# GlassyWing/yolo_deepsort

Measured on AMD Instinct MI355X. Metric: end-to-end frames/sec (detect+ReID+assoc), 608x608, higher is better.
Workload: dtype f16x3

## Files before the change

include/ydsort.h:

```cpp
#ifndef YDSORT_H
#define YDSORT_H

#include <stddef.h>
#include <stdint.h>

#ifdef __cplusplus
extern "C" {
#endif

typedef struct yds_net yds_net;
typedef struct yds_reid yds_reid;
typedef struct yds_trk yds_trk;
typedef struct yds_pipe yds_pipe;
typedef struct yds_comm yds_comm;

int yds_init(int device_id);
int yds_current_device(void);
int yds_device_pci_bus_id(char *buf, int len);
const char *yds_last_error(void);
int yds_device_count(void);
const char *yds_build_info(void);
void *yds_host_alloc(size_t nbytes);
int yds_host_free(void *host);
void *yds_dev_alloc(size_t nbytes);
// ... 13 lines not shown
int yds_darknet_num_boxes(const yds_net *);
int yds_darknet_num_attrs(const yds_net *);
int yds_darknet_num_layers(const yds_net *);
int yds_darknet_layer_shape(const yds_net *, int layer, int *c, int *h, int *w);
int64_t yds_darknet_conv_flops(const yds_net *);
int yds_darknet_forward_f32(yds_net *, const float *nchw_host, int batch, float *out_host);
int yds_darknet_forward_u8(yds_net *, const uint8_t *rgb_hwc_host, int h, int w, int batch,
                           float *out_host_or_null);
int yds_darknet_forward_u8_dev(yds_net *, const uint8_t *rgb_hwc_dev, int h, int w, int batch);
const uint8_t *yds_darknet_last_frames_dev(yds_net *, int *h, int *w, int *batch);
int yds_darknet_layer_output(yds_net *, int layer, int batch, float *nchw_host);
int yds_darknet_get_input(yds_net *, int batch, float *nchw_host);

int yds_nms(yds_net *, int image, float conf_thres, float iou_thres, int frame_h, int frame_w,
            float *out6_host, int cap, int *n_out);
int yds_nms_pred(const float *pred_host, int n_boxes, int attrs, float conf_thres, float iou_thres,
                 float *out6_host, int cap, int *n_out);

int yds_detect_tiled(yds_net *, const uint8_t *rgb_hwc_host, int h, int w, const int32_t *tiles_xyhw, int n_tiles,
                     float conf_thres, float iou_thres, float *out6_host, int cap, int *n_out);
int yds_nms_merge_pred(const float *pred_host, int n_boxes, int attrs, float conf_thres, float iou_thres,
                       float *out6_host, int cap, int *n_out);
int yds_nms_merge_pred_batched(const float *pred_host, int n_frames, int n_boxes, int attrs, float conf_thres, float iou_thres,
                               float *out6_host, int cap, int *n_out);

yds_reid *yds_reid_create(int max_crops);
void yds_reid_destroy(yds_reid *);
int yds_reid_load_tensor(yds_reid *, const char *name, const float *data_host, const int64_t *shape, int ndim);
int yds_reid_finalize(yds_reid *);
int64_t yds_reid_flops_per_crop(void);
// ... 110 lines not shown
```

yolo_deepsort_amd/_lib.py:

```python

from __future__ import annotations

import ctypes as C
import os

import numpy as np

HERE = os.path.dirname(os.path.abspath(__file__))
_TAG = os.environ.get("YDS_BUILD_TAG", "")
LIB_PATH = os.path.join(HERE, "libydsort" + ("_" + _TAG if _TAG else "") + ".so")


class YdsError(RuntimeError):
    pass


_P = C.c_void_p
_I = C.c_int
_F = C.c_float
_SZ = C.c_size_t
_I64 = C.c_int64

SIGNATURES = {
    "yds_init": (_I, [_I]),
# ... 28 lines not shown
    "yds_darknet_last_frames_dev": (_P, [_P, _P, _P, _P]),
    "yds_darknet_layer_output": (_I, [_P, _I, _I, _P]),
    "yds_darknet_get_input": (_I, [_P, _I, _P]),
    "yds_darknet_set_injection": (_I, [_P, _I, _P, _I, _F]),
    "yds_darknet_load_injection_sets": (_I, [_P, _P, _P, _I, _F]),
    "yds_darknet_select_injection_set": (_I, [_P, _I]),
    "yds_conv_variant_name": (C.c_char_p, [_I]),
    "yds_conv_timing_ex": (_I, [_P, _I, _P, _P, _P, _P, _P]),
    "yds_conv_num_variants": (_I, []),
    "yds_conv_clock": (_I, [_P, _P, _I]),
    "yds_set_conv_math": (_I, [_I]),
    "yds_get_conv_math": (_I, []),
    "yds_conv_bench": (_I, [_I, _I, _I, _I, _I, _I, _I, _I, _I, _I, _P, _P]),
    "yds_conv_run": (_I, [_I, _I, _I, _I, _I, _I, _I, _I, _I, _I, _P, _P, _P, _P, _P]),
    "yds_nms": (_I, [_P, _I, _F, _F, _I, _I, _P, _I, _P]),
    "yds_nms_pred": (_I, [_P, _I, _I, _F, _F, _P, _I, _P]),
    "yds_nms_merge_pred": (_I, [_P, _I, _I, _F, _F, _P, _I, _P]),
    "yds_nms_merge_pred_batched": (_I, [_P, _I, _I, _I, _F, _F, _P, _I, _P]),
    "yds_detect_tiled": (_I, [_P, _P, _I, _I, _P, _I, _F, _F, _P, _I, _P]),
    "yds_reid_create": (_P, [_I]),
    "yds_reid_destroy": (None, [_P]),
    "yds_reid_load_tensor": (_I, [_P, C.c_char_p, _P, _P, _I]),
    "yds_reid_finalize": (_I, [_P]),
    "yds_reid_flops_per_crop": (_I64, []),
    "yds_reid_embed": (_I, [_P, _P, _I, _I, _P, _I, _P]),
    "yds_reid_embed_dev": (_I, [_P, _P, _I, _I, _P, _I, _P]),
    "yds_reid_features_dev": (_P, [_P]),
    "yds_reid_preprocess": (_I, [_P, _P, _I, _I, _P, _I, _P]),
    "yds_reid_forward_f32": (_I, [_P, _P, _I, _P]),
    "yds_tracker_create": (_P, [C.c_double, C.c_double, _I, _I, _I]),
# ... 205 lines not shown
```

yolo_deepsort_amd/csrc/common.h:

```cpp
#pragma once
#include <hip/hip_runtime.h>
#include <stdint.h>
#include <stdio.h>
#include <string>
#include <vector>
#include <stdexcept>

namespace yds {

void set_error(const std::string &msg);
struct Error : std::runtime_error {
    explicit Error(const std::string &m) : std::runtime_error(m) {}
};
[[noreturn]] void fail(const char *fmt, ...);
int bound_device();
void bind_thread();
hipStream_t make_stream(bool latency_role);

#define YDS_HIP(expr)                                                                          \
    do {                                                                                       \
        hipError_t _e = (expr);                                                                \
        if (_e != hipSuccess)                                                                  \
            ::yds::fail("%s failed: %s (%s:%d)", #expr, hipGetErrorString(_e), __FILE__, __LINE__); \
    } while (0)
// ... 79 lines not shown
int conv_math();
void set_conv_math(int m);
void pack_weights_f16x3(const float *w, int cout, int kpad, std::vector<uint16_t> &out);
const char *conv_variant_name(int v);
double conv_flops(const ConvArgs &a);
double conv_bytes_io(const View &v);
double conv_bytes(const ConvArgs &a);

void launch_maxpool(const View &x, const View &y, int k, int stride, int pad, bool zero_pad_br, hipStream_t s);
void launch_upsample(const View &x, const View &y, int stride, hipStream_t s);
void launch_copy(const View &x, const View &y, hipStream_t s);
void launch_add(const View &a, const View &b, const View &y, hipStream_t s);
void launch_nchw_to_nhwc(const float *src_nchw, const View &y, int c_src, hipStream_t s);
void launch_nhwc_to_nchw(const View &x, float *dst_nchw, hipStream_t s);
void launch_pack_h16(const float *src_f32, const View &y, hipStream_t s);
void launch_yolo_decode(const View &head, float *out, int total_boxes, int box_off, int num_classes,
                        const float *anchors_wh , int A, int img_h, int img_w, hipStream_t s);
void launch_inject(const View &head, int image, const float *rows_dev, int n, int head_index, int num_classes,
                   float logit, hipStream_t s);
void launch_inject_batch(const View &head, int batch, const float *table_dev, const int *offsets_dev, int max_rows, int head_index,
                         int num_classes, float logit, hipStream_t s);
void launch_resize_u8(const uint8_t *frames, int n, int h, int w, const View &y, hipStream_t s, bool bgr = false);
void launch_window_resize(const uint8_t *frames, int h, int w, const int *tiles_dev, int T, int slot0, int n, const View &y, hipStream_t s,
                          bool bgr);
void launch_window_boxes(const float *pred, int n_boxes, int attrs, const int *tiles_dev, const float *scale_dev, int T, int slot0, int n,
                         float *dst, hipStream_t s);
void launch_crop_resize(const uint8_t *frames, int h, int w, const int *boxes5_dev, int D, const View &y,
                        hipStream_t s, bool bgr = false);
void launch_avgpool_l2norm(const View &x, float *out, hipStream_t s);

// ... 2 lines not shown
```

yolo_deepsort_amd/csrc/darknet.cpp:

```cpp
#include "engine.h"
#include "h16.h"
#include "conv_common.h"

#include <math.h>
#include <stdlib.h>
#include <string.h>
#include <map>
#include <sstream>

namespace yds {

std::vector<CfgBlock> parse_cfg(const std::string &text) {
    std::vector<CfgBlock> blocks;
    std::istringstream in(text);
    std::string line;
    auto strip = [](std::string s) {
        size_t a = s.find_first_not_of(" \t\r\n"), b = s.find_last_not_of(" \t\r\n");
        return a == std::string::npos ? std::string() : s.substr(a, b - a + 1);
    };
    while (std::getline(in, line)) {
        if (line.empty() || line[0] == '#') continue;
        line = strip(line);
        if (line.empty()) fail("cfg: whitespace-only line (the reference parser rejects it too)");
        if (line[0] == '[') {
// ... 277 lines not shown
    plan_half_formats();
    stem_checked_reset();
}

void Darknet::allocate_buffers() {
    size_t total_floats = 0;
    for (size_t i = 0; i < layers.size(); ++i) {
        if (!storage[i].owns) continue;
        const Layer &l = layers[i];
        size_t n = (size_t)batch_max * l.h * l.w * storage[i].ld;
        storage[i].buf.alloc(n);
        YDS_HIP(hipMemsetAsync(storage[i].buf.p, 0, n * sizeof(float), stream));
        total_floats += n;
    }
    input.alloc((size_t)batch_max * img_h * img_w * 4);
    out.alloc((size_t)batch_max * total_boxes * attrs);
    stage_f32.alloc((size_t)batch_max * img_h * img_w * 4);
    activation_bytes = total_floats * sizeof(float);
    YDS_HIP(hipStreamSynchronize(stream));
    inject_rows.clear();
    inject_rows.resize(batch_max);
    inject_n.assign(batch_max, 0);
    inject_active = false;
    inject_offsets.clear();
    inject_set = -1;
    stem_checked = block1_checked = -1;
    stage_n = 0;
}

void Darknet::set_batch_max(int b) {
    if (b < 1) fail("set_batch_max: %d", b);
// ... 21 lines not shown
        return v;
    }
    const Storage &st = storage[r];
    if (st.redirected) {
        const Storage &dst = storage[st.into];
        v.fmt = half_mode ? dst.fmt_half : dst.fmt;
        v.p = dst.buf.p + fmt_slots(v.fmt, st.coff + l.coff);
        v.ld = fmt_slots(v.fmt, dst.ld);
    } else {
        v.fmt = half_mode ? st.fmt_half : st.fmt;
        v.p = st.buf.p + fmt_slots(v.fmt, l.coff);
        v.ld = fmt_slots(v.fmt, st.ld);
    }
    v.p += (size_t)lane_img0 * l.h * l.w * v.ld;
    return v;
}

View Darknet::input_view(int batch) const {
    View v;
    v.p = input.p + (size_t)lane_img0 * img_h * img_w * 4; v.n = batch; v.h = img_h; v.w = img_w; v.c = 4; v.ld = 4;
    return v;
}

size_t Darknet::weight_floats() const {
    size_t n = 0;
    for (const Layer &l : layers)
        if (l.type == "convolutional") n += (size_t)(l.bn ? 4 : 1) * l.c + (size_t)l.c * l.cin_file * l.ksize * l.ksize;
    return n;
}

// ... 212 lines not shown
        } else if (l.type == "route") {
            if (l.refs.size() > 1) {
                View dst = view(i, batch);
                for (auto &cp : l.copies) {
                    View d = dst;
                    d.p += fmt_slots(dst.fmt, cp.second);
                    launch_copy(view(cp.first, batch), d, stream);
                }
            }
        } else if (l.type == "shortcut") {
            if (!l.fused) launch_add(view(l.refs[0], batch), view(l.refs[1], batch), view(i, batch), stream);
        } else if (l.type == "yolo") {
            View head = view(l.src, batch);
            int hidx = 0;
            for (int y : yolo_layers) { if (y == i) break; ++hidx; }
            if (hidx == 0 && out_guard) YDS_HIP(hipStreamWaitEvent(stream, out_guard, 0));
            if (inject_active && inject_set >= 0) {
                launch_inject_batch(head, batch, inject_table.p, inject_offsets_dev.p + (size_t)inject_set * batch_max + first, inject_max_rows, hidx,
                                    l.classes, inject_logit, stream);
            } else {
                for (int b = 0; b < batch && inject_active; ++b)
                    launch_inject(head, b, inject_rows[first + b].p, inject_n[first + b], hidx, l.classes, inject_logit, stream);
            }
            launch_yolo_decode(head, out.p + (size_t)first * total_boxes * attrs, total_boxes, l.box_off, l.classes, l.anchors.data(), (int)l.anchors.size() / 2, img_h, img_w, stream);
        }
    }
}

void Darknet::forward_f32_host(const float *nchw, int batch, float *out_host) {
    size_t n = (size_t)batch * in_channels * img_h * img_w;
    YDS_HIP(hipMemcpyAsync(stage_f32.p, nchw, n * sizeof(float), hipMemcpyHostToDevice, stream));
    launch_nchw_to_nhwc(stage_f32.p, input_view(batch), in_channels, stream);
    run_graph(batch);
    if (out_host) YDS_HIP(hipMemcpyAsync(out_host, out.p, (size_t)batch * total_boxes * attrs * sizeof(float), hipMemcpyDeviceToHost, stream));
    YDS_HIP(hipStreamSynchronize(stream));
}

void Darknet::forward_u8_dev(const uint8_t *frames_dev, int h, int w, int batch) {
    if (in_channels != 3) fail("forward_u8: network expects %d channels", in_channels);
// ... 412 lines not shown
```

yolo_deepsort_amd/csrc/engine.h:

```cpp
#pragma once
#include "common.h"

#include <map>
#include <memory>
#include <string>
#include <utility>
#include <vector>

namespace yds {

struct CfgBlock {
    std::string type;
    std::map<std::string, std::string> kv;
};
std::vector<CfgBlock> parse_cfg(const std::string &text);

struct Layer {
    std::string type;
    int c = 0, h = 0, w = 0;
    int root = -1, coff = 0;
    bool is_view = false;
    int src = -1;
    std::vector<int> refs;
    std::vector<std::pair<int, int>> copies;
// ... 16 lines not shown
    DevBuf<float> buf;
    int ld = 0;
    int fmt = 0;
    int fmt_half = 0;
    bool owns = false;
    bool redirected = false;
    int into = -1, coff = 0;
};

struct WindowTable {
    DevBuf<int> rects;
    DevBuf<float> scale;
    int T = 0;
    void build(const int *rects_xyhw, int n, int img_h, int img_w, hipStream_t s);
    std::vector<float> scale_host;
};

class Darknet {
public:
    Darknet(const std::string &cfg_text, int img_h, int img_w, int batch_max);
    ~Darknet();
    void load_weights(const void *blob, size_t nbytes, int cutoff);
    void set_batch_max(int b);
    void forward_f32_host(const float *nchw, int batch, float *out_host);
    void forward_u8_host(const uint8_t *frames, int h, int w, int batch, float *out_host);
    void forward_u8_dev(const uint8_t *frames_dev, int h, int w, int batch);
    void forward_resized(int batch) { run_graph(batch); }
    bool forward_resized_part(int batch, int part);
    int head_layers() const;
    void forward_tiles_host(const uint8_t *frame, int h, int w, const int *tiles_xyhw, int n_tiles);
// ... 8 lines not shown
    int64_t flops_per_image() const;
    size_t weight_floats() const;
    View view(int layer, int batch) const;
    ConvArgs conv_args(int layer, int batch) const;
    ConvArgs merged_conv_args(int layer, int batch) const;
    View input_view(int batch) const;

    int img_h, img_w, batch_max, in_channels = 3;
    int math = 0;
    bool half_mode = false;
    void stem_checked_reset() { stem_checked = block1_checked = -1; }
    void set_half(bool on);
    void plan_half_formats();
    int owner_of(int layer, int &off) const;
    int total_boxes = 0, attrs = 0;
    std::vector<Layer> layers;
    std::vector<Storage> storage;
    std::vector<int> yolo_layers;
    DevBuf<float> input, out, stage_f32;
    DevBuf<uint8_t> stage_u8;
    int stage_h = 0, stage_w = 0, stage_n = 0;
    DevBuf<float> tiled_pred;
    WindowTable tiles;
    hipStream_t stream = nullptr;
    int32_t header[5] = {0, 0, 0, 0, 0};
    bool weights_loaded = false;
    size_t activation_bytes = 0;
    std::vector<DevBuf<float>> inject_rows;
    std::vector<int> inject_n;
    bool inject_active = false;
// ... 24 lines not shown
    bool block1_fused(int batch);
    hipEvent_t out_guard = nullptr;
    int lane_img0 = 0;
    std::vector<hipStream_t> lane_streams;
    std::vector<hipEvent_t> lane_done;
    hipEvent_t lane_fork = nullptr;
};

class NmsWorkspace {
public:
    explicit NmsWorkspace(int max_candidates = 16384, int frames = 1);
    ~NmsWorkspace();
    NmsWorkspace(const NmsWorkspace &) = delete;
    void launch(const float *pred_dev, size_t pred_stride, int n_frames, int n_boxes, int attrs, float conf_thres, float iou_thres,
                float sx, float sy, int cap, hipStream_t s, bool corner = false, bool merge = false);
    int collect(int frame, float *out6_host, int cap);
    void resize(int max_candidates, int n_frames);
    int needed(int n_frames) const;
    static constexpr int kMaxCandidates = 1 << 18;
    int run(const float *pred_dev, int n_boxes, int attrs, float conf_thres, float iou_thres, float sx, float sy,
            float *out6_host, int cap, hipStream_t s);
    int run_merge(const float *pred_dev, int n_boxes, int attrs, float conf_thres, float iou_thres, float *out6_host, int cap, hipStream_t s);
    int max_cand, frames;
    DevBuf<float> cand;
    DevBuf<float> sorted;
    DevBuf<int> counts;
    DevBuf<int> box_count;
    DevBuf<unsigned long long> mask;
    DevBuf<float> kept;
    DevBuf<int> order;
    int *h_counts = nullptr;
    float *h_kept = nullptr;
};

class ReidNet {
public:
    explicit ReidNet(int max_crops);
    ~ReidNet();
    void load_tensor(const std::string &name, const float *data, const int64_t *shape, int ndim);
    void finalize();
    void embed_dev(const uint8_t *frame_dev, int h, int w, const float *tlwh_host, int D, float *out_host);
    void embed_multi_dev(const uint8_t *frames_dev, int h, int w, const float *tlwh_host, const int *frame_of, int D, bool bgr = false);
    void embed_host(const uint8_t *frame_host, int h, int w, const float *tlwh_host, int D, float *out_host);
    void preprocess_host(const uint8_t *frame_host, int h, int w, const float *tlwh_host, int D, float *nchw_host);
    void forward_f32_host(const float *nchw, int D, float *out_host);
    void forward(int D);
    void reserve(int D);
// ... 48 lines not shown
```

yolo_deepsort_amd/csrc/layers.hip:

```cpp
#include "common.h"

#include <algorithm>
#include "h16.h"

namespace yds {

static inline int grid_for(size_t work, int block = 256) {
    size_t g = (work + block - 1) / block;
    if (g > 8192) g = 8192;
    if (g < 1) g = 1;
    return (int)g;
}

__global__ void maxpool_kernel(const float *x, float *y, int N, int H, int W, int C, int ldx, int Ho, int Wo, int ldy,
                               int k, int stride, int pad, int zero_br, int fmt_in, int fmt_out) {
    fp16_saturate_on();
    const int C4 = C >> 2;
    const size_t total = (size_t)N * Ho * Wo * C4;
    for (size_t idx = blockIdx.x * (size_t)blockDim.x + threadIdx.x; idx < total; idx += (size_t)gridDim.x * blockDim.x) {
        int c4 = idx % C4;
        size_t pix = idx / C4;
        int ox = pix % Wo;
        size_t t = pix / Wo;
        int oy = t % Ho;
// ... 147 lines not shown
        const float v[4] = {t.x, t.y, t.z, t.w};
        h16_store4(y + pix * ldy, c4 * 4, v);
    }
}
void launch_pack_h16(const float *src_f32, const View &y, hipStream_t s) {
    if (y.c % 32 || y.ld % 32) fail("pack_h16: channels must be a multiple of 32");
    hipLaunchKernelGGL(pack_h16_kernel, dim3(grid_for(y.pixels() * (y.c / 4))), dim3(256), 0, s, src_f32, y.p, y.pixels(), y.c, y.ld);
    YDS_HIP(hipGetLastError());
}

void launch_nhwc_to_nchw(const View &x, float *dst_nchw, hipStream_t s) {
    hipLaunchKernelGGL(nhwc_to_nchw_kernel, dim3(grid_for(x.pixels() * x.c)), dim3(256), 0, s, x.p, dst_nchw, x.n, x.c, x.h, x.w, x.ld, x.fmt);
    YDS_HIP(hipGetLastError());
}

struct YoloParams {
    float aw[8], ah[8];
    float s0, s1;
};

__global__ void yolo_decode_kernel(const float *head, float *out, int N, int H, int W, int ld, int A, int attrs, int total_boxes,
                                   int box_off, YoloParams yp) {
    const int HW = H * W, n = blockIdx.y, per_cell = A * attrs;
    (void)N;
    const int lane = threadIdx.x & 63;
    const int wave0 = __builtin_amdgcn_readfirstlane((int)((blockIdx.x * blockDim.x + threadIdx.x) >> 6));
    const int nwaves = (int)((gridDim.x * blockDim.x) >> 6);
    for (int cell = wave0; cell < HW; cell += nwaves) {
        const int gy = cell / W, gx = cell - gy * W;
        const float *src = head + ((size_t)(n * H + gy) * W + gx) * ld;
        float *dst = out + ((size_t)n * total_boxes + box_off + cell) * attrs;
        for (int i = lane; i < per_cell; i += 64) {
            int a = 0;
#pragma unroll
            for (int k = 1; k < 8; ++k) a += (k < A && i >= k * attrs) ? 1 : 0;
            const int t = i - a * attrs;
            const float v = src[i];
            float r;
            if (t == 0) r = __fmul_rn(__fadd_rn(1.f / (1.f + expf(-v)), (float)gx), yp.s0);
            else if (t == 1) r = __fmul_rn(__fadd_rn(1.f / (1.f + expf(-v)), (float)gy), yp.s1);
            else if (t == 2) r = __fmul_rn(__fmul_rn(expf(v), yp.aw[a]), yp.s0);
            else if (t == 3) r = __fmul_rn(__fmul_rn(expf(v), yp.ah[a]), yp.s1);
            else r = 1.f / (1.f + expf(-v));
            dst[(size_t)a * HW * attrs + t] = r;
        }
    }
}

void launch_yolo_decode(const View &head, float *out, int total_boxes, int box_off, int num_classes, const float *anchors_wh,
                        int A, int img_h, int img_w, hipStream_t s) {
    if (A > 8) fail("yolo: at most 8 anchors per head");
    YoloParams yp;
    yp.s0 = (float)((double)img_h / head.h);
    yp.s1 = (float)((double)img_w / head.w);
    for (int a = 0; a < A; ++a) {
        yp.aw[a] = anchors_wh[2 * a] / yp.s0;
        yp.ah[a] = anchors_wh[2 * a + 1] / yp.s1;
    }
    int attrs = num_classes + 5;
    if (head.c != A * attrs) fail("yolo: head has %d channels, expected %d", head.c, A * attrs);
    const size_t per_img = (size_t)A * head.h * head.w * attrs;
    if (per_img >= (1ull << 31)) fail("yolo: head too large for 32-bit indexing");
    const unsigned cells = (unsigned)head.h * head.w;
    hipLaunchKernelGGL(yolo_decode_kernel, dim3(std::min((cells + 3) / 4, 2048u), head.n), dim3(256), 0, s, head.p, out, head.n, head.h, head.w,
                       head.ld, A, attrs, total_boxes, box_off, yp);
    YDS_HIP(hipGetLastError());
}

__global__ void inject_clear_kernel(float *head, int image, int H, int W, int ld, int A, int attrs, float logit) {
    int total = H * W * A;
    for (int idx = blockIdx.x * blockDim.x + threadIdx.x; idx < total; idx += gridDim.x * blockDim.x) {
        int a = idx % A, cell = idx / A;
        head[((size_t)image * H * W + cell) * ld + a * attrs + 4] = -logit;
// ... 255 lines not shown
```

yolo_deepsort_amd/csrc/nms.hip:

```cpp
#include "engine.h"

#include <string.h>

#include <algorithm>
#include <vector>

namespace yds {

constexpr int MAX_DET = 300;

__global__ void nms_count_kernel(const float *pred_all, size_t pred_stride, int n_boxes, int attrs, float thr, int *box_count_all) {
    const float *pred = pred_all + blockIdx.y * pred_stride;
    int *box_count = box_count_all + (size_t)blockIdx.y * n_boxes;
    int i = blockIdx.x * blockDim.x + threadIdx.x;
    if (i >= n_boxes) return;
    const float *p = pred + (size_t)i * attrs;
    int cnt = 0;
    float obj = p[4];
    if (obj > thr) {
        for (int j = 5; j < attrs; ++j) cnt += __fmul_rn(p[j], obj) > thr;
    }
    box_count[i] = cnt;
}

__global__ void nms_scan_kernel(int *box_count_all, int n_boxes, int *counts_all) {
    int *box_count = box_count_all + (size_t)blockIdx.y * n_boxes;
    int *counts = counts_all + blockIdx.y * 4;
    __shared__ int wave_sum[16];
    __shared__ int carry;
    const int tid = threadIdx.x, lane = tid & 63, wave = tid >> 6;
    if (tid == 0) carry = 0;
    __syncthreads();
    for (int base = 0; base < n_boxes; base += blockDim.x) {
        int i = base + tid;
        int v = i < n_boxes ? box_count[i] : 0;
// ... 3 lines not shown
            if (lane >= o) incl += t;
        }
        if (lane == 63) wave_sum[wave] = incl;
        __syncthreads();
        int woff = 0;
        for (int w = 0; w < wave; ++w) woff += wave_sum[w];
        int c = carry;
        if (i < n_boxes) box_count[i] = c + woff + incl - v;
        __syncthreads();
        if (tid == (int)blockDim.x - 1) carry = c + woff + incl;
        __syncthreads();
    }
    if (tid == 0) { counts[0] = carry; counts[1] = 0; }
}

__global__ void nms_emit_kernel(const float *pred_all, size_t pred_stride, int n_boxes, int attrs, float thr, const int *box_off_all, int max_cand,
                                float *cand_all, int corner) {
    const float *pred = pred_all + blockIdx.y * pred_stride;
    const int *box_off = box_off_all + (size_t)blockIdx.y * n_boxes;
    float *cand = cand_all + (size_t)blockIdx.y * max_cand * 6;
    int i = blockIdx.x * blockDim.x + threadIdx.x;
    if (i >= n_boxes) return;
    const float *p = pred + (size_t)i * attrs;
    float obj = p[4];
    if (!(obj > thr)) return;
    int slot = box_off[i];
    float x1 = p[0], y1 = p[1], x2 = p[2], y2 = p[3];
    if (!corner) {
        float hw = __fdiv_rn(p[2], 2.f), hh = __fdiv_rn(p[3], 2.f);
        x1 = __fsub_rn(p[0], hw); y1 = __fsub_rn(p[1], hh); x2 = __fadd_rn(p[0], hw); y2 = __fadd_rn(p[1], hh);
    }
    for (int j = 5; j < attrs; ++j) {
        float sc = __fmul_rn(p[j], obj);
        if (sc > thr) {
            if (slot < max_cand) {
                float *r = cand + (size_t)slot * 6;
                r[0] = x1; r[1] = y1; r[2] = x2; r[3] = y2; r[4] = sc; r[5] = (float)(j - 5);
            }
            ++slot;
        }
    }
}

__global__ void nms_rank_kernel(const float *cand_all, const int *counts_all, int max_cand, float *sorted_all) {
    const float *cand = cand_all + (size_t)blockIdx.y * max_cand * 6;
    float *sorted = sorted_all + (size_t)blockIdx.y * max_cand * 6;
    const int *counts = counts_all + blockIdx.y * 4;
    __shared__ float tile[256];
// ... 158 lines not shown
        mean[threadIdx.x] = __fdiv_rn((float)acc, wsum);
    }
    __syncthreads();
    for (int i = threadIdx.x; i < k * 4; i += blockDim.x) kept[(size_t)(i >> 2) * 6 + (i & 3)] = mean[i & 3];
}

__global__ __launch_bounds__(256) void nms_publish_kernel(const int *counts, const float *kept, int *h_counts, float *h_kept, int cap) {
    const int f = blockIdx.x;
    if (threadIdx.x < 4) h_counts[f * 4 + threadIdx.x] = counts[f * 4 + threadIdx.x];
    const int n = min(counts[f * 4 + 1], cap) * 6;
    const float *src = kept + (size_t)f * MAX_DET * 6;
    float *dst = h_kept + (size_t)f * MAX_DET * 6;
    for (int i = threadIdx.x; i < n; i += 256) dst[i] = src[i];
}

void NmsWorkspace::launch(const float *pred_dev, size_t pred_stride, int n_frames, int n_boxes, int attrs, float conf_thres, float iou_thres,
                          float sx, float sy, int cap, hipStream_t s, bool corner, bool merge) {
    if (attrs < 6) fail("nms: predictions need at least one class");
    if (n_frames < 1) fail("nms: no frames");
    if (n_frames > frames) resize(max_cand, n_frames);
    box_count.ensure((size_t)frames * n_boxes);
    const int nb = (n_boxes + 255) / 256;
    hipLaunchKernelGGL(nms_count_kernel, dim3(nb, n_frames), dim3(256), 0, s, pred_dev, pred_stride, n_boxes, attrs, conf_thres, box_count.p);
    hipLaunchKernelGGL(nms_scan_kernel, dim3(1, n_frames), dim3(1024), 0, s, box_count.p, n_boxes, counts.p);
    hipLaunchKernelGGL(nms_emit_kernel, dim3(nb, n_frames), dim3(256), 0, s, pred_dev, pred_stride, n_boxes, attrs, conf_thres, box_count.p,
                       max_cand, cand.p, corner ? 1 : 0);
    hipLaunchKernelGGL(nms_rank_kernel, dim3(16, n_frames), dim3(256), 0, s, cand.p, counts.p, max_cand, sorted.p);
    const int words_ld = max_cand / 64;
    hipLaunchKernelGGL(nms_mask_kernel, dim3(64, n_frames), dim3(256), 0, s, sorted.p, counts.p, max_cand, (double)iou_thres, mask.p, words_ld);
    hipLaunchKernelGGL(nms_sweep_kernel, dim3(1, n_frames), dim3(256), words_ld * sizeof(unsigned long long), s, sorted.p, mask.p, words_ld,
                       counts.p, max_cand, sx, sy, kept.p, cap);
    if (merge) hipLaunchKernelGGL(nms_merge_kernel, dim3(n_frames), dim3(256), 0, s, cand.p, sorted.p, counts.p, max_cand, iou_thres, kept.p);
    hipLaunchKernelGGL(nms_publish_kernel, dim3(n_frames), dim3(256), 0, s, counts.p, kept.p, h_counts, h_kept, std::min(cap, (int)MAX_DET));
    YDS_HIP(hipGetLastError());
}

int NmsWorkspace::collect(int frame, float *out6_host, int cap) {
    const int *c = h_counts + frame * 4;
    if (c[0] > max_cand) fail("nms: %d candidates exceed the workspace capacity %d (caller must resize and relaunch)", c[0], max_cand);
    int n = c[1] < cap ? c[1] : cap;
    if (n > 0) memcpy(out6_host, h_kept + (size_t)frame * MAX_DET * 6, (size_t)n * 6 * sizeof(float));
    return n;
}

int NmsWorkspace::run(const float *pred_dev, int n_boxes, int attrs, float conf_thres, float iou_thres, float sx, float sy,
                      float *out6_host, int cap, hipStream_t s) {
    launch(pred_dev, 0, 1, n_boxes, attrs, conf_thres, iou_thres, sx, sy, cap, s);
    YDS_HIP(hipStreamSynchronize(s));
    if (needed(1) > max_cand) {
// ... 54 lines not shown
yds::NmsWorkspace &workspace() {
    static thread_local std::unique_ptr<yds::NmsWorkspace> ws;
    if (!ws) ws.reset(new yds::NmsWorkspace());
    return *ws;
}
}

extern "C" {

int yds_nms(yds_net *n, int image, float conf_thres, float iou_thres, int frame_h, int frame_w, float *out6_host, int cap, int *n_out) {
    YDS_API_BEGIN
    yds::Darknet *d = n->d;
    if (image < 0 || image >= d->batch_max) yds::fail("nms: image %d outside batch", image);
    float sx = frame_h > 0 ? (float)((double)frame_w / d->img_w) : 1.f;
    float sy = frame_h > 0 ? (float)((double)frame_h / d->img_h) : 1.f;
    const float *pred = d->out.p + (size_t)image * d->total_boxes * d->attrs;
    *n_out = workspace().run(pred, d->total_boxes, d->attrs, conf_thres, iou_thres, sx, sy, out6_host, cap, d->stream);
    YDS_API_END
}

int yds_detect_tiled(yds_net *n, const uint8_t *rgb_hwc_host, int h, int w, const int32_t *tiles_xyhw, int n_tiles, float conf_thres,
                     float iou_thres, float *out6_host, int cap, int *n_out) {
    YDS_API_BEGIN
    yds::Darknet *d = n->d;
    d->forward_tiles_host(rgb_hwc_host, h, w, tiles_xyhw, n_tiles);
    *n_out = workspace().run_merge(d->tiled_pred.p, n_tiles * d->total_boxes, d->attrs, conf_thres, iou_thres, out6_host, cap, d->stream);
    YDS_API_END
}

int yds_nms_merge_pred(const float *pred_host, int n_boxes, int attrs, float conf_thres, float iou_thres, float *out6_host, int cap, int *n_out) {
    YDS_API_BEGIN
    yds::DevBuf<float> pred;
// ... 37 lines not shown
```

yolo_deepsort_amd/csrc/pipeline.cpp:

```cpp
#include "engine.h"

#include <limits.h>
#include <stdlib.h>

#include <chrono>
#include <utility>

namespace yds {

struct DetSlot {
    std::unique_ptr<NmsWorkspace> nms;
    hipEvent_t e0, e1, e2, e_nms;
    hipEvent_t e_r0, e_r1;
    bool reid_in_pass = false;
    DetSlot() { for (hipEvent_t *e : {&e0, &e1, &e2, &e_nms, &e_r0, &e_r1}) YDS_HIP(hipEventCreate(e)); }
    ~DetSlot() { for (hipEvent_t e : {e0, e1, e2, e_nms, e_r0, e_r1}) (void)hipEventDestroy(e); }
};

struct Pass {
    const uint8_t *frames = nullptr;
    int h = 0, w = 0, batch = 0;
    int slot = 0;
    enum { NOTHING, HEAD, WHOLE } done = NOTHING;
    bool split = false;
// ... 73 lines not shown
        hipEvent_t up_done = nullptr;
        Read rd[2];
        Slot() { for (hipEvent_t *e : {&up_done, &rd[DET].ev, &rd[REID].ev}) YDS_HIP(hipEventCreateWithFlags(e, hipEventDisableTiming)); }
        ~Slot() { for (hipEvent_t e : {up_done, rd[DET].ev, rd[REID].ev}) (void)hipEventDestroy(e); }
    };
    Slot slots[N];
    int turn = 0;
    hipStream_t copy_stream = nullptr, det_stream, reid_stream;
};

class Pipeline {
public:
    Pipeline(Darknet *net, ReidNet *reid, std::vector<TrackerIface *> trks, bool multi, float conf, float nms_iou, const int32_t *mask, int n_mask)
        : net(net), reid(reid), trks(std::move(trks)), group(make_tracker_group()), multi(multi), conf(conf), nms_thres(nms_iou),
          class_mask(mask, mask + n_mask), deep_min(getenv("YDS_PIPE_DEEP_MIN") ? atoi(getenv("YDS_PIPE_DEEP_MIN")) : 64),
          stager(net->stream, reid->stream) {
        for (DetSlot &s : det) s.nms.reset(new NmsWorkspace(4096, net->batch_max));
        YDS_HIP(hipEventCreateWithFlags(&ev_feat, hipEventDisableTiming));
        YDS_HIP(hipEventCreateWithFlags(&ev_reid_done, hipEventDisableTiming));
    }
    ~Pipeline() {
        (void)hipEventDestroy(ev_feat);
        (void)hipEventDestroy(ev_reid_done);
    }

    void prefetch_host(const uint8_t *frames_host, int h, int w, int batch) {
        if (stager.find(frames_host) >= 0) return;
        stager.upload(frames_host, (size_t)batch * h * w * 3, 3, stager.cur, stager.next);
    }
    void step_host(const uint8_t *frames_host, const uint8_t *next_host, int h, int w, int batch, int32_t *out6, int cap, int32_t *counts) {
// ... 28 lines not shown
    }
    void launch_detector_tail(Pass &p) {
        DetSlot &s = det[p.slot];
        const size_t per_slot = (size_t)net->total_boxes * net->attrs;
        if (const int T = windows_for(p.h, p.w)) {
            if (win_pred.n < (size_t)p.batch * T * per_slot) {
                YDS_HIP(hipStreamSynchronize(net->stream));
                win_pred.alloc((size_t)p.batch * T * per_slot);
            }
            net->forward_windows(p.frames, p.h, p.w, p.batch, win, win_pred.p, frames_bgr);
            stager.mark_read(p.frames, net->stream, FrameStager::DET);
            YDS_HIP(hipEventRecord(s.e2, net->stream));
            s.nms->launch(win_pred.p, (size_t)T * per_slot, p.batch, T * net->total_boxes, net->attrs, conf, nms_thres, 1.f, 1.f, 300, net->stream,
                          true, true);
        } else {
            if (p.split) (void)net->forward_resized_part(p.batch, 1);
            else net->forward_resized(p.batch);
            YDS_HIP(hipEventRecord(s.e2, net->stream));
            const float sx = (float)((double)p.w / net->img_w), sy = (float)((double)p.h / net->img_h);
            s.nms->launch(net->out.p, per_slot, p.batch, net->total_boxes, net->attrs, conf, nms_thres, sx, sy, 300, net->stream);
        }
        YDS_HIP(hipEventRecord(s.e_nms, net->stream));
        p.done = Pass::WHOLE;
    }

    void set_windows(int ww, int wh, double overlap) {
        if (pending.frames || ahead.reid_in_flight) fail("pipeline: set_windows while a look-ahead pass is in flight (consume it with a step first)");
        if (ww > 0 && wh <= 0) fail("pipeline: window %d x %d", ww, wh);
        if (ww > 0 && !(overlap >= 0)) fail("pipeline: window overlap %g", overlap);
        win_w = ww > 0 ? ww : 0; win_h = ww > 0 ? wh : 0; win_overlap = overlap;
        win_tab_h = win_tab_w = 0;
    }
    int windows_for(int h, int w) {
        if (win_w <= 0 || (w < win_w && h < win_h)) return 0;
        if (h == win_tab_h && w == win_tab_w) return win.T;
// ... 172 lines not shown
        for (int b = 0; b < n; ++b)
            if (stream_of_frame[b] < 0 || stream_of_frame[b] >= (int)trks.size())
                fail("pipeline: frame %d belongs to stream %d outside [0,%zu)", b, stream_of_frame[b], trks.size());
        stream_of.assign(stream_of_frame, stream_of_frame + n);
    }

    Darknet *net;
    ReidNet *reid;
    std::vector<TrackerIface *> trks;
    std::unique_ptr<TrackerGroupIface> group;
    const bool multi;
    std::vector<int32_t> stream_of;
    float conf, nms_thres;
    std::vector<int32_t> class_mask;
    const int deep_min;
    DetSlot det[2];
    Pass pending;
    FrameStager stager;
    Dets cur, ahead;
    DevBuf<float> feat_cur;
    int next_inject_set = -1;
    hipEvent_t ev_feat = nullptr;
    int schedule_min_crops = INT_MIN;
    Trial trials[2];
    hipEvent_t ev_reid_done = nullptr;
    hipStream_t reid_last_on = nullptr;
    bool last_serial = false;
    bool frames_bgr = false;
    float stage_us[5] = {0, 0, 0, 0, 0};
    int win_w = 0, win_h = 0, win_tab_h = 0, win_tab_w = 0;
// ... 111 lines not shown
```

yolo_deepsort_amd/models.py:

```python

from __future__ import annotations

import ctypes as C

import numpy as np

from . import _lib
from .loaders import parse_model_config


def _to_numpy(x):
    if hasattr(x, "detach"):
        x = x.detach().cpu().numpy()
    return np.ascontiguousarray(x, dtype=np.float32)


class _Param:

    def __init__(self, device):
        self.device = device


class Darknet:
    def __init__(self, config_path, img_size=416, batch_max=1, cfg_text=None):
# ... 107 lines not shown
            self.set_batch_max(b)
        out = np.empty((b, self.num_boxes, self.num_attrs), np.float32) if want_output else None
        _lib.check(_lib.load().yds_darknet_forward_u8(self._h, _lib.ptr(frames), h, w, b, _lib.ptr(out)))
        return out

    def last_frame_dev(self, frame):
        if getattr(self, "_last_frame_src", None) is not frame:
            return None
        h, w, b = C.c_int(), C.c_int(), C.c_int()
        p = _lib.load().yds_darknet_last_frames_dev(self._h, C.byref(h), C.byref(w), C.byref(b))
        if not p or b.value != 1 or (h.value, w.value) != tuple(frame.shape[:2]):
            return None
        return C.c_void_p(p)

    def nms(self, image, conf_thres, iou_thres, frame_hw=None, cap=300):
        out = np.empty((cap, 6), np.float32)
        n = C.c_int(0)
        fh, fw = frame_hw if frame_hw is not None else (0, 0)
        _lib.check(_lib.load().yds_nms(self._h, image, conf_thres, iou_thres, fh, fw, _lib.ptr(out), cap, C.byref(n)))
        return out[:n.value].copy()

    def detect_tiled(self, frame, tiles, conf_thres, iou_thres, cap=300):
        frame = np.ascontiguousarray(frame, dtype=np.uint8)
        h, w, _ = frame.shape
        rects = np.ascontiguousarray(tiles, dtype=np.int32).reshape(-1, 4)
        out = np.empty((cap, 6), np.float32)
        n = C.c_int(0)
        _lib.check(_lib.load().yds_detect_tiled(self._h, _lib.ptr(frame), h, w, _lib.ptr(rects), rects.shape[0], conf_thres, iou_thres,
                                                _lib.ptr(out), cap, C.byref(n)))
        return out[:n.value].copy()

    def layer_shape(self, i):
        c, h, w = C.c_int(), C.c_int(), C.c_int()
        _lib.check(_lib.load().yds_darknet_layer_shape(self._h, i, C.byref(c), C.byref(h), C.byref(w)))
# ... 48 lines not shown
```

Measured before the change: 1675.

## Fuse YOLO head decode into NMS candidate kernels, skipping dense decode buffer

```diff
diff --git a/include/ydsort.h b/include/ydsort.h
--- a/include/ydsort.h
+++ b/include/ydsort.h
@@ -51,6 +51,8 @@
 
 int yds_nms(yds_net *, int image, float conf_thres, float iou_thres, int frame_h, int frame_w,
             float *out6_host, int cap, int *n_out);
+int yds_nms_heads(yds_net *, int image, float conf_thres, float iou_thres, int frame_h, int frame_w,
+                  float *out6_host, int cap, int *n_out);
 int yds_nms_pred(const float *pred_host, int n_boxes, int attrs, float conf_thres, float iou_thres,
                  float *out6_host, int cap, int *n_out);
 
diff --git a/yolo_deepsort_amd/_lib.py b/yolo_deepsort_amd/_lib.py
--- a/yolo_deepsort_amd/_lib.py
+++ b/yolo_deepsort_amd/_lib.py
@@ -66,6 +66,7 @@
     "yds_conv_bench": (_I, [_I, _I, _I, _I, _I, _I, _I, _I, _I, _I, _P, _P]),
     "yds_conv_run": (_I, [_I, _I, _I, _I, _I, _I, _I, _I, _I, _I, _P, _P, _P, _P, _P]),
     "yds_nms": (_I, [_P, _I, _F, _F, _I, _I, _P, _I, _P]),
+    "yds_nms_heads": (_I, [_P, _I, _F, _F, _I, _I, _P, _I, _P]),
     "yds_nms_pred": (_I, [_P, _I, _I, _F, _F, _P, _I, _P]),
     "yds_nms_merge_pred": (_I, [_P, _I, _I, _F, _F, _P, _I, _P]),
     "yds_nms_merge_pred_batched": (_I, [_P, _I, _I, _I, _F, _F, _P, _I, _P]),
diff --git a/yolo_deepsort_amd/csrc/common.h b/yolo_deepsort_amd/csrc/common.h
--- a/yolo_deepsort_amd/csrc/common.h
+++ b/yolo_deepsort_amd/csrc/common.h
@@ -117,6 +117,11 @@
 void launch_nchw_to_nhwc(const float *src_nchw, const View &y, int c_src, hipStream_t s);
 void launch_nhwc_to_nchw(const View &x, float *dst_nchw, hipStream_t s);
 void launch_pack_h16(const float *src_f32, const View &y, hipStream_t s);
+struct YoloParams {
+    float aw[8], ah[8];
+    float s0, s1;
+};
+YoloParams yolo_params(const View &head, const float *anchors_wh , int A, int img_h, int img_w);
 void launch_yolo_decode(const View &head, float *out, int total_boxes, int box_off, int num_classes,
                         const float *anchors_wh , int A, int img_h, int img_w, hipStream_t s);
 void launch_inject(const View &head, int image, const float *rows_dev, int n, int head_index, int num_classes,
diff --git a/yolo_deepsort_amd/csrc/darknet.cpp b/yolo_deepsort_amd/csrc/darknet.cpp
--- a/yolo_deepsort_amd/csrc/darknet.cpp
+++ b/yolo_deepsort_amd/csrc/darknet.cpp
@@ -315,7 +315,8 @@
         total_floats += n;
     }
     input.alloc((size_t)batch_max * img_h * img_w * 4);
-    out.alloc((size_t)batch_max * total_boxes * attrs);
+    out.release();
+    heads_written = false;
     stage_f32.alloc((size_t)batch_max * img_h * img_w * 4);
     activation_bytes = total_floats * sizeof(float);
     YDS_HIP(hipStreamSynchronize(stream));
@@ -367,6 +368,23 @@
     }
     v.p += (size_t)lane_img0 * l.h * l.w * v.ld;
     return v;
+}
+
+bool Darknet::head_table(YoloHeads &t) const {
+    t = YoloHeads();
+    if (yolo_layers.empty() || (int)yolo_layers.size() > YoloHeads::kMax) return false;
+    for (int y : yolo_layers) {
+        const Layer &l = layers[y];
+        View v = view(l.src, 1);
+        const int A = (int)l.anchors.size() / 2;
+        if (v.fmt != FMT_F32 || A > 8 || v.c != A * attrs) return false;
+        v.p -= (size_t)lane_img0 * l.h * l.w * v.ld;
+        YoloHead &h = t.head[t.n++];
+        h.p = v.p; h.h = v.h; h.w = v.w; h.ld = v.ld; h.A = A; h.box_off = l.box_off;
+        h.yp = yolo_params(v, l.anchors.data(), A, img_h, img_w);
+    }
+    t.attrs = attrs; t.total_boxes = total_boxes;
+    return true;
 }
 
 View Darknet::input_view(int batch) const {
@@ -609,7 +627,7 @@
             View head = view(l.src, batch);
             int hidx = 0;
             for (int y : yolo_layers) { if (y == i) break; ++hidx; }
-            if (hidx == 0 && out_guard) YDS_HIP(hipStreamWaitEvent(stream, out_guard, 0));
+            if (decode_dense && hidx == 0 && out_guard) YDS_HIP(hipStreamWaitEvent(stream, out_guard, 0));
             if (inject_active && inject_set >= 0) {
                 launch_inject_batch(head, batch, inject_table.p, inject_offsets_dev.p + (size_t)inject_set * batch_max + first, inject_max_rows, hidx,
                                     l.classes, inject_logit, stream);
@@ -617,7 +635,11 @@
                 for (int b = 0; b < batch && inject_active; ++b)
                     launch_inject(head, b, inject_rows[first + b].p, inject_n[first + b], hidx, l.classes, inject_logit, stream);
             }
-            launch_yolo_decode(head, out.p + (size_t)first * total_boxes * attrs, total_boxes, l.box_off, l.classes, l.anchors.data(), (int)l.anchors.size() / 2, img_h, img_w, stream);
+            if (decode_dense) {
+                out.ensure((size_t)batch_max * total_boxes * attrs);
+                launch_yolo_decode(head, out.p + (size_t)first * total_boxes * attrs, total_boxes, l.box_off, l.classes, l.anchors.data(), (int)l.anchors.size() / 2, img_h, img_w, stream);
+            }
+            heads_written = true;
         }
     }
 }
diff --git a/yolo_deepsort_amd/csrc/engine.h b/yolo_deepsort_amd/csrc/engine.h
--- a/yolo_deepsort_amd/csrc/engine.h
+++ b/yolo_deepsort_amd/csrc/engine.h
@@ -54,6 +54,17 @@
     int T = 0;
     void build(const int *rects_xyhw, int n, int img_h, int img_w, hipStream_t s);
     std::vector<float> scale_host;
+};
+
+struct YoloHead {
+    const float *p = nullptr;
+    int h = 0, w = 0, ld = 0, A = 0, box_off = 0;
+    YoloParams yp;
+};
+struct YoloHeads {
+    static constexpr int kMax = 4;
+    YoloHead head[kMax];
+    int n = 0, attrs = 0, total_boxes = 0;
 };
 
 class Darknet {
@@ -92,6 +103,9 @@
     void plan_half_formats();
     int owner_of(int layer, int &off) const;
     int total_boxes = 0, attrs = 0;
+    bool decode_dense = true;
+    bool heads_written = false;
+    bool head_table(YoloHeads &t) const;
     std::vector<Layer> layers;
     std::vector<Storage> storage;
     std::vector<int> yolo_layers;
@@ -146,6 +160,7 @@
     NmsWorkspace(const NmsWorkspace &) = delete;
     void launch(const float *pred_dev, size_t pred_stride, int n_frames, int n_boxes, int attrs, float conf_thres, float iou_thres,
                 float sx, float sy, int cap, hipStream_t s, bool corner = false, bool merge = false);
+    void launch_heads(const YoloHeads &heads, int n_frames, float conf_thres, float iou_thres, float sx, float sy, int cap, hipStream_t s);
     int collect(int frame, float *out6_host, int cap);
     void resize(int max_candidates, int n_frames);
     int needed(int n_frames) const;
@@ -163,6 +178,10 @@
     DevBuf<int> order;
     int *h_counts = nullptr;
     float *h_kept = nullptr;
+
+private:
+    template <class Src> void launch_from(const Src &src, int n_frames, float conf_thres, float iou_thres, float sx, float sy, int cap,
+                                          hipStream_t s, bool corner, bool merge);
 };
 
 class ReidNet {
diff --git a/yolo_deepsort_amd/csrc/layers.hip b/yolo_deepsort_amd/csrc/layers.hip
--- a/yolo_deepsort_amd/csrc/layers.hip
+++ b/yolo_deepsort_amd/csrc/layers.hip
@@ -2,6 +2,7 @@
 
 #include <algorithm>
 #include "h16.h"
+#include "yolo_decode.h"
 
 namespace yds {
 
@@ -185,11 +186,6 @@
     YDS_HIP(hipGetLastError());
 }
 
-struct YoloParams {
-    float aw[8], ah[8];
-    float s0, s1;
-};
-
 __global__ void yolo_decode_kernel(const float *head, float *out, int N, int H, int W, int ld, int A, int attrs, int total_boxes,
                                    int box_off, YoloParams yp) {
     const int HW = H * W, n = blockIdx.y, per_cell = A * attrs;
@@ -207,27 +203,26 @@
             for (int k = 1; k < 8; ++k) a += (k < A && i >= k * attrs) ? 1 : 0;
             const int t = i - a * attrs;
             const float v = src[i];
-            float r;
-            if (t == 0) r = __fmul_rn(__fadd_rn(1.f / (1.f + expf(-v)), (float)gx), yp.s0);
-            else if (t == 1) r = __fmul_rn(__fadd_rn(1.f / (1.f + expf(-v)), (float)gy), yp.s1);
-            else if (t == 2) r = __fmul_rn(__fmul_rn(expf(v), yp.aw[a]), yp.s0);
-            else if (t == 3) r = __fmul_rn(__fmul_rn(expf(v), yp.ah[a]), yp.s1);
-            else r = 1.f / (1.f + expf(-v));
-            dst[(size_t)a * HW * attrs + t] = r;
+            dst[(size_t)a * HW * attrs + t] = yolo_decode_value(t, v, gx, gy, a, yp);
         }
     }
 }
 
-void launch_yolo_decode(const View &head, float *out, int total_boxes, int box_off, int num_classes, const float *anchors_wh,
-                        int A, int img_h, int img_w, hipStream_t s) {
+YoloParams yolo_params(const View &head, const float *anchors_wh, int A, int img_h, int img_w) {
     if (A > 8) fail("yolo: at most 8 anchors per head");
-    YoloParams yp;
+    YoloParams yp = {};
     yp.s0 = (float)((double)img_h / head.h);
     yp.s1 = (float)((double)img_w / head.w);
     for (int a = 0; a < A; ++a) {
         yp.aw[a] = anchors_wh[2 * a] / yp.s0;
         yp.ah[a] = anchors_wh[2 * a + 1] / yp.s1;
     }
+    return yp;
+}
+
+void launch_yolo_decode(const View &head, float *out, int total_boxes, int box_off, int num_classes, const float *anchors_wh,
+                        int A, int img_h, int img_w, hipStream_t s) {
+    const YoloParams yp = yolo_params(head, anchors_wh, A, img_h, img_w);
     int attrs = num_classes + 5;
     if (head.c != A * attrs) fail("yolo: head has %d channels, expected %d", head.c, A * attrs);
     const size_t per_img = (size_t)A * head.h * head.w * attrs;
diff --git a/yolo_deepsort_amd/csrc/nms.hip b/yolo_deepsort_amd/csrc/nms.hip
--- a/yolo_deepsort_amd/csrc/nms.hip
+++ b/yolo_deepsort_amd/csrc/nms.hip
@@ -1,4 +1,5 @@
 #include "engine.h"
+#include "yolo_decode.h"
 
 #include <string.h>
 
@@ -9,16 +10,53 @@
 
 constexpr int MAX_DET = 300;
 
-__global__ void nms_count_kernel(const float *pred_all, size_t pred_stride, int n_boxes, int attrs, float thr, int *box_count_all) {
-    const float *pred = pred_all + blockIdx.y * pred_stride;
+struct DenseRows {
+    const float *pred;
+    size_t stride;
+    int n_boxes, n_attrs;
+    struct Row {
+        const float *p;
+        __device__ __forceinline__ float obj() const { return p[4]; }
+        __device__ __forceinline__ float cls(int j) const { return p[j]; }
+        __device__ __forceinline__ float box(int k) const { return p[k]; }
+    };
+    __host__ __device__ __forceinline__ int boxes() const { return n_boxes; }
+    __host__ __device__ __forceinline__ int attrs() const { return n_attrs; }
+    __device__ __forceinline__ Row row(int frame, int i) const { return Row{pred + frame * stride + (size_t)i * n_attrs}; }
+};
+struct HeadRows {
+    YoloHeads t;
+    struct Row {
+        const float *p;
+        const YoloHead *head;
+        int gx, gy, a;
+        __device__ __forceinline__ float obj() const { return yolo_sigmoid(p[4]); }
+        __device__ __forceinline__ float cls(int j) const { return yolo_sigmoid(p[j]); }
+        __device__ __forceinline__ float box(int k) const { return yolo_decode_value(k, p[k], gx, gy, a, head->yp); }
+    };
+    __host__ __device__ __forceinline__ int boxes() const { return t.total_boxes; }
+    __host__ __device__ __forceinline__ int attrs() const { return t.attrs; }
+    __device__ __forceinline__ Row row(int frame, int i) const {
+        int h = 0;
+#pragma unroll
+        for (int k = 1; k < YoloHeads::kMax; ++k) h += (k < t.n && i >= t.head[k].box_off) ? 1 : 0;
+        const YoloHead *hd = &t.head[h];
+        const int HW = hd->h * hd->w, r = i - hd->box_off;
+        const int a = r / HW, cell = r - a * HW, gy = cell / hd->w;
+        return Row{hd->p + ((size_t)frame * HW + cell) * hd->ld + a * t.attrs, hd, cell - gy * hd->w, gy, a};
+    }
+};
+
+template <class Src> __global__ void nms_count_kernel(Src src, float thr, int *box_count_all) {
+    const int n_boxes = src.boxes(), attrs = src.attrs();
     int *box_count = box_count_all + (size_t)blockIdx.y * n_boxes;
     int i = blockIdx.x * blockDim.x + threadIdx.x;
     if (i >= n_boxes) return;
-    const float *p = pred + (size_t)i * attrs;
+    const typename Src::Row p = src.row(blockIdx.y, i);
     int cnt = 0;
-    float obj = p[4];
+    float obj = p.obj();
     if (obj > thr) {
-        for (int j = 5; j < attrs; ++j) cnt += __fmul_rn(p[j], obj) > thr;
+        for (int j = 5; j < attrs; ++j) cnt += __fmul_rn(p.cls(j), obj) > thr;
     }
     box_count[i] = cnt;
 }
@@ -52,24 +90,24 @@
     if (tid == 0) { counts[0] = carry; counts[1] = 0; }
 }
 
-__global__ void nms_emit_kernel(const float *pred_all, size_t pred_stride, int n_boxes, int attrs, float thr, const int *box_off_all, int max_cand,
-                                float *cand_all, int corner) {
-    const float *pred = pred_all + blockIdx.y * pred_stride;
+template <class Src> __global__ void nms_emit_kernel(Src src, float thr, const int *box_off_all, int max_cand, float *cand_all, int corner) {
+    const int n_boxes = src.boxes(), attrs = src.attrs();
     const int *box_off = box_off_all + (size_t)blockIdx.y * n_boxes;
     float *cand = cand_all + (size_t)blockIdx.y * max_cand * 6;
     int i = blockIdx.x * blockDim.x + threadIdx.x;
     if (i >= n_boxes) return;
-    const float *p = pred + (size_t)i * attrs;
-    float obj = p[4];
+    const typename Src::Row p = src.row(blockIdx.y, i);
+    float obj = p.obj();
     if (!(obj > thr)) return;
     int slot = box_off[i];
-    float x1 = p[0], y1 = p[1], x2 = p[2], y2 = p[3];
+    const float b0 = p.box(0), b1 = p.box(1), b2 = p.box(2), b3 = p.box(3);
+    float x1 = b0, y1 = b1, x2 = b2, y2 = b3;
     if (!corner) {
-        float hw = __fdiv_rn(p[2], 2.f), hh = __fdiv_rn(p[3], 2.f);
-        x1 = __fsub_rn(p[0], hw); y1 = __fsub_rn(p[1], hh); x2 = __fadd_rn(p[0], hw); y2 = __fadd_rn(p[1], hh);
+        float hw = __fdiv_rn(b2, 2.f), hh = __fdiv_rn(b3, 2.f);
+        x1 = __fsub_rn(b0, hw); y1 = __fsub_rn(b1, hh); x2 = __fadd_rn(b0, hw); y2 = __fadd_rn(b1, hh);
     }
     for (int j = 5; j < attrs; ++j) {
-        float sc = __fmul_rn(p[j], obj);
+        float sc = __fmul_rn(p.cls(j), obj);
         if (sc > thr) {
             if (slot < max_cand) {
                 float *r = cand + (size_t)slot * 6;
@@ -258,17 +296,17 @@
     for (int i = threadIdx.x; i < n; i += 256) dst[i] = src[i];
 }
 
-void NmsWorkspace::launch(const float *pred_dev, size_t pred_stride, int n_frames, int n_boxes, int attrs, float conf_thres, float iou_thres,
-                          float sx, float sy, int cap, hipStream_t s, bool corner, bool merge) {
+template <class Src> void NmsWorkspace::launch_from(const Src &src, int n_frames, float conf_thres, float iou_thres, float sx, float sy, int cap,
+                                                    hipStream_t s, bool corner, bool merge) {
+    const int n_boxes = src.boxes(), attrs = src.attrs();
     if (attrs < 6) fail("nms: predictions need at least one class");
     if (n_frames < 1) fail("nms: no frames");
     if (n_frames > frames) resize(max_cand, n_frames);
     box_count.ensure((size_t)frames * n_boxes);
     const int nb = (n_boxes + 255) / 256;
-    hipLaunchKernelGGL(nms_count_kernel, dim3(nb, n_frames), dim3(256), 0, s, pred_dev, pred_stride, n_boxes, attrs, conf_thres, box_count.p);
+    hipLaunchKernelGGL(nms_count_kernel<Src>, dim3(nb, n_frames), dim3(256), 0, s, src, conf_thres, box_count.p);
     hipLaunchKernelGGL(nms_scan_kernel, dim3(1, n_frames), dim3(1024), 0, s, box_count.p, n_boxes, counts.p);
-    hipLaunchKernelGGL(nms_emit_kernel, dim3(nb, n_frames), dim3(256), 0, s, pred_dev, pred_stride, n_boxes, attrs, conf_thres, box_count.p,
-                       max_cand, cand.p, corner ? 1 : 0);
+    hipLaunchKernelGGL(nms_emit_kernel<Src>, dim3(nb, n_frames), dim3(256), 0, s, src, conf_thres, box_count.p, max_cand, cand.p, corner ? 1 : 0);
     hipLaunchKernelGGL(nms_rank_kernel, dim3(16, n_frames), dim3(256), 0, s, cand.p, counts.p, max_cand, sorted.p);
     const int words_ld = max_cand / 64;
     hipLaunchKernelGGL(nms_mask_kernel, dim3(64, n_frames), dim3(256), 0, s, sorted.p, counts.p, max_cand, (double)iou_thres, mask.p, words_ld);
@@ -277,6 +315,16 @@
     if (merge) hipLaunchKernelGGL(nms_merge_kernel, dim3(n_frames), dim3(256), 0, s, cand.p, sorted.p, counts.p, max_cand, iou_thres, kept.p);
     hipLaunchKernelGGL(nms_publish_kernel, dim3(n_frames), dim3(256), 0, s, counts.p, kept.p, h_counts, h_kept, std::min(cap, (int)MAX_DET));
     YDS_HIP(hipGetLastError());
+}
+
+void NmsWorkspace::launch(const float *pred_dev, size_t pred_stride, int n_frames, int n_boxes, int attrs, float conf_thres, float iou_thres,
+                          float sx, float sy, int cap, hipStream_t s, bool corner, bool merge) {
+    launch_from(DenseRows{pred_dev, pred_stride, n_boxes, attrs}, n_frames, conf_thres, iou_thres, sx, sy, cap, s, corner, merge);
+}
+
+void NmsWorkspace::launch_heads(const YoloHeads &heads, int n_frames, float conf_thres, float iou_thres, float sx, float sy, int cap, hipStream_t s) {
+    if (heads.n < 1 || heads.n > YoloHeads::kMax) fail("nms: head table of %d yolo layers", heads.n);
+    launch_from(HeadRows{heads}, n_frames, conf_thres, iou_thres, sx, sy, cap, s, false, false);
 }
 
 int NmsWorkspace::collect(int frame, float *out6_host, int cap) {
@@ -361,8 +409,30 @@
     if (image < 0 || image >= d->batch_max) yds::fail("nms: image %d outside batch", image);
     float sx = frame_h > 0 ? (float)((double)frame_w / d->img_w) : 1.f;
     float sy = frame_h > 0 ? (float)((double)frame_h / d->img_h) : 1.f;
+    if (!d->out.p) yds::fail("nms: this network has not run a dense decode (no forward yet, or only passes that left the head tensors: yds_nms_heads)");
     const float *pred = d->out.p + (size_t)image * d->total_boxes * d->attrs;
     *n_out = workspace().run(pred, d->total_boxes, d->attrs, conf_thres, iou_thres, sx, sy, out6_host, cap, d->stream);
+    YDS_API_END
+}
+
+int yds_nms_heads(yds_net *n, int image, float conf_thres, float iou_thres, int frame_h, int frame_w, float *out6_host, int cap, int *n_out) {
+    YDS_API_BEGIN
+    yds::Darknet *d = n->d;
+    if (image < 0 || image >= d->batch_max) yds::fail("nms: image %d outside batch", image);
+    yds::YoloHeads heads;
+    if (!d->head_table(heads)) yds::fail("nms: this network's heads are read through the dense decode only (yds_nms)");
+    if (!d->heads_written) yds::fail("nms: this network has not run a forward yet (its head tensors hold nothing)");
+    for (int h = 0; h < heads.n; ++h) heads.head[h].p += (size_t)image * heads.head[h].h * heads.head[h].w * heads.head[h].ld;
+    float sx = frame_h > 0 ? (float)((double)frame_w / d->img_w) : 1.f;
+    float sy = frame_h > 0 ? (float)((double)frame_h / d->img_h) : 1.f;
+    yds::NmsWorkspace &ws = workspace();
+    for (int pass = 0; pass < 2; ++pass) {
+        ws.launch_heads(heads, 1, conf_thres, iou_thres, sx, sy, cap, d->stream);
+        YDS_HIP(hipStreamSynchronize(d->stream));
+        if (ws.needed(1) <= ws.max_cand) break;
+        ws.resize(ws.needed(1), ws.frames);
+    }
+    *n_out = ws.collect(0, out6_host, cap);
     YDS_API_END
 }
 
diff --git a/yolo_deepsort_amd/csrc/pipeline.cpp b/yolo_deepsort_amd/csrc/pipeline.cpp
--- a/yolo_deepsort_amd/csrc/pipeline.cpp
+++ b/yolo_deepsort_amd/csrc/pipeline.cpp
@@ -111,6 +111,7 @@
     Pipeline(Darknet *net, ReidNet *reid, std::vector<TrackerIface *> trks, bool multi, float conf, float nms_iou, const int32_t *mask, int n_mask)
         : net(net), reid(reid), trks(std::move(trks)), group(make_tracker_group()), multi(multi), conf(conf), nms_thres(nms_iou),
           class_mask(mask, mask + n_mask), deep_min(getenv("YDS_PIPE_DEEP_MIN") ? atoi(getenv("YDS_PIPE_DEEP_MIN")) : 64),
+          dense_decode(getenv("YDS_DENSE_DECODE") && atoi(getenv("YDS_DENSE_DECODE")) != 0),
           stager(net->stream, reid->stream) {
         for (DetSlot &s : det) s.nms.reset(new NmsWorkspace(4096, net->batch_max));
         YDS_HIP(hipEventCreateWithFlags(&ev_feat, hipEventDisableTiming));
@@ -169,11 +170,18 @@
             s.nms->launch(win_pred.p, (size_t)T * per_slot, p.batch, T * net->total_boxes, net->attrs, conf, nms_thres, 1.f, 1.f, 300, net->stream,
                           true, true);
         } else {
-            if (p.split) (void)net->forward_resized_part(p.batch, 1);
-            else net->forward_resized(p.batch);
+            YoloHeads heads;
+            const bool sparse = !dense_decode && net->head_table(heads);
+            {
+                struct Restore { bool &v; bool keep; ~Restore() { v = keep; } } restore{net->decode_dense, net->decode_dense};
+                net->decode_dense = !sparse;
+                if (p.split) (void)net->forward_resized_part(p.batch, 1);
+                else net->forward_resized(p.batch);
+            }
             YDS_HIP(hipEventRecord(s.e2, net->stream));
             const float sx = (float)((double)p.w / net->img_w), sy = (float)((double)p.h / net->img_h);
-            s.nms->launch(net->out.p, per_slot, p.batch, net->total_boxes, net->attrs, conf, nms_thres, sx, sy, 300, net->stream);
+            if (sparse) s.nms->launch_heads(heads, p.batch, conf, nms_thres, sx, sy, 300, net->stream);
+            else s.nms->launch(net->out.p, per_slot, p.batch, net->total_boxes, net->attrs, conf, nms_thres, sx, sy, 300, net->stream);
         }
         YDS_HIP(hipEventRecord(s.e_nms, net->stream));
         p.done = Pass::WHOLE;
@@ -376,6 +384,7 @@
     float conf, nms_thres;
     std::vector<int32_t> class_mask;
     const int deep_min;
+    const bool dense_decode;
     DetSlot det[2];
     Pass pending;
     FrameStager stager;
diff --git a/yolo_deepsort_amd/csrc/yolo_decode.h b/yolo_deepsort_amd/csrc/yolo_decode.h
--- /dev/null
+++ b/yolo_deepsort_amd/csrc/yolo_decode.h
@@ -0,0 +1,18 @@
+#pragma once
+#include "common.h"
+
+namespace yds {
+
+__device__ __forceinline__ float yolo_sigmoid(float v) { return 1.f / (1.f + expf(-v)); }
+
+__device__ __forceinline__ float yolo_decode_value(int t, float v, int gx, int gy, int a, const YoloParams &yp) {
+    float r;
+    if (t == 0) r = __fmul_rn(__fadd_rn(yolo_sigmoid(v), (float)gx), yp.s0);
+    else if (t == 1) r = __fmul_rn(__fadd_rn(yolo_sigmoid(v), (float)gy), yp.s1);
+    else if (t == 2) r = __fmul_rn(__fmul_rn(expf(v), yp.aw[a]), yp.s0);
+    else if (t == 3) r = __fmul_rn(__fmul_rn(expf(v), yp.ah[a]), yp.s1);
+    else r = yolo_sigmoid(v);
+    return r;
+}
+
+}
diff --git a/yolo_deepsort_amd/models.py b/yolo_deepsort_amd/models.py
--- a/yolo_deepsort_amd/models.py
+++ b/yolo_deepsort_amd/models.py
@@ -145,10 +145,16 @@
         return C.c_void_p(p)
 
     def nms(self, image, conf_thres, iou_thres, frame_hw=None, cap=300):
+        return self._nms(_lib.load().yds_nms, image, conf_thres, iou_thres, frame_hw, cap)
+
+    def nms_heads(self, image, conf_thres, iou_thres, frame_hw=None, cap=300):
+        return self._nms(_lib.load().yds_nms_heads, image, conf_thres, iou_thres, frame_hw, cap)
+
+    def _nms(self, fn, image, conf_thres, iou_thres, frame_hw, cap):
         out = np.empty((cap, 6), np.float32)
         n = C.c_int(0)
         fh, fw = frame_hw if frame_hw is not None else (0, 0)
-        _lib.check(_lib.load().yds_nms(self._h, image, conf_thres, iou_thres, fh, fw, _lib.ptr(out), cap, C.byref(n)))
+        _lib.check(fn(self._h, image, conf_thres, iou_thres, fh, fw, _lib.ptr(out), cap, C.byref(n)))
         return out[:n.value].copy()
 
     def detect_tiled(self, frame, tiles, conf_thres, iou_thres, cap=300):
```

After: 1696, median of 5. 1.01x the previous value.
